# urbste/MultiCol-SLAM

Hardware: NVIDIA B200
Metric: Mfeatures/s extract+match (higher is better)
Workload: dtype u8

## Files before the change

multicol_slam_b200/csrc/describe_kernel.cu:

```cuda
#include <cstdlib>
#include <cstring>
#include <vector>

#include "cam_model.cuh"
#include "kernels.h"
#include "mcs_common.cuh"

namespace mcs {

__constant__ signed char c_pairs[2048];
__device__ float2 g_patf[1024];
__constant__ signed char c_disc_u[848], c_disc_v[848];

__device__ __forceinline__ float fast_atan2_deg(float y, float x) {
    const float s = (float)(180.0 / 3.14159265358979323846);
    const float p1 = 0.9997878412794807f * s, p3 = -0.3258083974640975f * s;
    const float p5 = 0.1555786518463281f * s, p7 = -0.04432655554792128f * s;
    const float ax = fabsf(x), ay = fabsf(y);
    float a, c, c2;
    if (ax >= ay) {
        c = __fdiv_rn(ay, __fadd_rn(ax, (float)2.2204460492503131e-16));
        c2 = __fmul_rn(c, c);
        a = __fmul_rn(__fadd_rn(__fmul_rn(__fadd_rn(__fmul_rn(__fadd_rn(__fmul_rn(p7, c2), p5), c2), p3), c2), p1), c);
    } else {
// ... 233 lines not shown
                tu = (u - uk) - mu; tv = (v - vk) - mv;
                ru = (tu + kMagic) - kMagic; rv = (tv + kMagic) - kMagic;
                bad |= !(fabs(tu - ru) < 0.5 - kT1RepairGuard) || !(fabs(tv - rv) < 0.5 - kT1RepairGuard);
            }
            bad |= !(fabs(tu) < (double)kPatchR + 0.4) || !(fabs(tv) < (double)kPatchR + 0.4);
            int ix = (int)ru, iy = (int)rv;
            ix = min(max(ix, -kPatchR), kPatchR); iy = min(max(iy, -kPatchR), kPatchR);
            smp[e2] = patch[pofs + iy * kPatchS + ix];
        }
        out |= (unsigned)(smp[0] < smp[1]) << (j >> 1);
    }
    if (lane_valid && (bad || worst_tau >= __double2hiint(1.0))) *fail = 1;
    return out;
}

struct __align__(16) WarpCtx {
    float t1[16];
    double ukx, uky, a_base, ca[3], sa[3];
    const double* row;
    int kx, ky, oidx, b, level;
    uint32_t c;
    float angle;
};
template <int PPL , int MINB = MCS_K3_MINB>
__global__ void __launch_bounds__(kDescWarps * 32, MINB)
describe_kernel(const PyramidGeom* __restrict__ geom, const DescribeArgs args, const mcs_ocam* __restrict__ cams,
                const DistortLut* __restrict__ luts, const int* __restrict__ cam_of_image,
                const uint32_t* __restrict__ sel_xys, const int* __restrict__ sel_count,
                mcs_keypoint* __restrict__ kps_out, uint8_t* __restrict__ desc_out, uint8_t* __restrict__ dmask_out,
                int* __restrict__ counts_out, const int capacity, const int n_images) {
    __shared__ mcs_ocam s_cam[kDescWarps];
    __shared__ WarpCtx s_ctx[kDescWarps];
    __shared__ __align__(8) float2 s_patf[PPL * 32];
    extern __shared__ __align__(8) float2 s_park_dyn[];
    __shared__ __align__(16) uint8_t s_patch[kDescWarps][(2 * kPatchR + 1) * kPatchS];
    const int ds = geom->desc_size;
#pragma unroll
    for (int i = threadIdx.x; i < PPL * 32; i += kDescWarps * 32) s_patf[i] = g_patf[i];
    __syncthreads();

    const int lane = threadIdx.x & 31, wib = threadIdx.x >> 5;
    const int warp_global = (blockIdx.x * blockDim.x + threadIdx.x) >> 5;
    const int sel_total = geom->sel_total;
    const int b = warp_global / sel_total;
    if (b >= n_images) return;
    const int slot = warp_global - b * sel_total;
    const int L = geom->nlevels;
    int level = 0, off = 0;
    for (int l = 0; l < L; ++l)
        if (slot >= geom->lv[l].sel_off) level = l;
    for (int l = 0; l < level; ++l) off += sel_count[b * L + l];
    const LevelGeom& g = geom->lv[level];
    const int p = slot - g.sel_off;
    const int cnt = sel_count[b * L + level];
    if (slot == 0 && lane == 0) {
        int tot = 0;
        for (int l = 0; l < L; ++l) tot += sel_count[b * L + l];
        counts_out[b] = min(tot, capacity);
    }
    if (p >= cnt) return;
    const int oidx = off + p;
    if (oidx >= capacity) return;
    const uint32_t c = sel_xys[(size_t)b * sel_total + slot];
    const int kx = corner_x(c), ky = corner_y(c);
    const uint8_t* uimg = args.lvl[level] + (size_t)b * g.img_bytes;
    const uint8_t* bimg = args.blur[level] + (size_t)b * g.img_bytes;
    const int pitch = g.pitch;

    uint8_t* patch = s_patch[wib];
    const int x0 = (kx - kPatchR) & ~3;
    {
        const int half = lane >> 4, w = lane & 15;
        const uint32_t* gp = (const uint32_t*)(bimg + (size_t)(ky - kPatchR + half) * pitch + x0) + w;
        uint32_t* sp = (uint32_t*)(patch + half * kPatchS) + w;
#pragma unroll
        for (int k0 = 0; k0 < 26; k0 += 13) {
            uint32_t t[13];
#pragma unroll
            for (int k = 0; k < 13; ++k) {
                const int r = half + 2 * (k0 + k);
                t[k] = (w < 15 && r < 2 * kPatchR + 1) ? __ldg(gp + (size_t)(k0 + k) * (pitch / 2)) : 0u;
            }
#pragma unroll
            for (int k = 0; k < 13; ++k) {
                const int r = half + 2 * (k0 + k);
                if (w < 15 && r < 2 * kPatchR + 1) sp[(k0 + k) * (2 * kPatchS / 4)] = t[k];
            }
        }
    }
    const int pofs = kPatchR * kPatchS + (kx - x0);

    int m10 = 0, m01 = 0;
#if MCS_K3_V3
    {
        constexpr int kIcS = 40;
        uint8_t* ic = reinterpret_cast<uint8_t*>(s_park_dyn + wib * (PPL * 32));
        const int xs = (kx - kHalfPatch) & ~3;
        {
            const int rr = lane / 10, w = lane - rr * 10;
            const uint32_t* gp = (const uint32_t*)(uimg + (size_t)(ky - kHalfPatch + rr) * pitch + xs) + w;
            uint32_t* sp = (uint32_t*)(ic + rr * kIcS) + w;
            uint32_t t[11];
#pragma unroll
            for (int k = 0; k < 11; ++k) t[k] = (lane < 30) ? __ldg(gp + (size_t)k * 3 * (pitch / 4)) : 0u;
#pragma unroll
            for (int k = 0; k < 11; ++k) if (lane < 30) sp[k * 3 * (kIcS / 4)] = t[k];
        }
        __syncwarp();
        const int u = lane - kHalfPatch;
        const int au = u < 0 ? -u : u;
        const int vm = c_disc_u[au];
        const uint8_t* col = ic + kHalfPatch * kIcS + (kx - kHalfPatch - xs) + lane;
        int sum = col[0];
#pragma unroll
        for (int k = 1; k <= kHalfPatch; ++k) {
            const int a = col[k * kIcS], bb = col[-k * kIcS];
            if (vm >= k) { sum += a + bb; m01 += k * (a - bb); }
        }
        m10 = u * sum;
        const int um = c_disc_u[kHalfPatch];
        if (lane < 2 * um + 1) {
            const int v = lane - um;
            const int val = ic[(kHalfPatch + v) * kIcS + (kx - kHalfPatch - xs) + 2 * kHalfPatch];
            m10 += kHalfPatch * val;
            m01 += v * val;
        }
#pragma unroll
        for (int o = 16; o; o >>= 1) {
            m10 += __shfl_xor_sync(0xffffffffu, m10, o);
            m01 += __shfl_xor_sync(0xffffffffu, m01, o);
        }
        __syncwarp();
    }
#else
    {
        const uint8_t* ctr = uimg + (size_t)ky * pitch + kx;
        const int u = lane - kHalfPatch;
        const int au = u < 0 ? -u : u;
        const int vm = c_disc_u[au];
#pragma unroll 11
        for (int v = -kHalfPatch; v <= kHalfPatch; ++v) {
            const int val = (v >= -vm && v <= vm) ? (int)ctr[v * pitch + u] : 0;
            m10 += u * val;
            m01 += v * val;
        }
        if (lane < 2 * c_disc_u[kHalfPatch] + 1) {
            const int v = lane - c_disc_u[kHalfPatch];
            const int val = ctr[v * pitch + kHalfPatch];
            m10 += kHalfPatch * val;
            m01 += v * val;
        }
#pragma unroll
        for (int o = 16; o; o >>= 1) {
            m10 += __shfl_xor_sync(0xffffffffu, m10, o);
            m01 += __shfl_xor_sync(0xffffffffu, m01, o);
        }
    }
#endif
    const float angle = fast_atan2_deg((float)m01, (float)m10);

    WarpCtx& cx = s_ctx[wib];
    const int ci = cam_of_image[b];
    const bool masks = geom->learn_masks != 0, dbrief = geom->do_dbrief != 0 || masks;
    const int npat = masks ? 3 : 1;
    {
        double a0, s0, c0;
        if (masks) a0 = (double)__fdiv_rn(angle, 57.2957763671875f);
        else a0 = (double)__fmul_rn(angle, 0.01745329238474369f);
        sincos(a0, &s0, &c0);
        if (lane == 0) {
            cx.kx = kx; cx.ky = ky; cx.oidx = oidx; cx.b = b; cx.level = level; cx.c = c; cx.angle = angle; cx.a_base = a0;
            const double c20 = 0.93969262078590838405, s20 = 0.34202014332566873304;
            cx.ca[0] = c0; cx.sa[0] = s0;
            cx.ca[1] = fma(c0, c20, -s0 * s20); cx.sa[1] = fma(s0, c20, c0 * s20);
            cx.ca[2] = fma(c0, c20, s0 * s20);  cx.sa[2] = fma(s0, c20, -c0 * s20);
        }
    }
    constexpr int BPL = PPL / 16;
    unsigned v0[BPL], vdiff[BPL];
#pragma unroll
    for (int bb = 0; bb < BPL; ++bb) { v0[bb] = 0u; vdiff[bb] = 0u; }
    auto put = [&](int qi, unsigned e ) {
#pragma unroll
        for (int bb = 0; bb < BPL; ++bb) {
            const unsigned v = (e >> (8 * bb)) & 0xFFu;
            if (qi == 0) v0[bb] = v; else vdiff[bb] |= v ^ v0[bb];
        }
    };
    __syncwarp();
    if (!dbrief) {
        const double ca0 = cx.ca[0], sa0 = cx.sa[0];
        int ix[PPL], iy[PPL];
        bool far = false;
#pragma unroll
        for (int j = 0; j < PPL; ++j) {
            const float2 pp = s_patf[j * 32 + lane];
            const double px = (double)pp.x, py = (double)pp.y;
            ix[j] = __double2int_rn(px * ca0 - py * sa0);
            iy[j] = __double2int_rn(px * sa0 + py * ca0);
            far |= (unsigned)(ix[j] + kPatchR) > 2u * kPatchR || (unsigned)(iy[j] + kPatchR) > 2u * kPatchR;
        }
        if (__any_sync(0xffffffffu, far)) {
            put(0, orb_pattern_global<PPL>(s_patf, ca0, sa0, lane, bimg, uimg, &g, kx, ky));
        } else {
            unsigned e = 0;
#pragma unroll
            for (int bb = 0; bb < BPL; ++bb) {
#pragma unroll
                for (int bit = 0; bit < 8; ++bit) {
                    const int j0 = 16 * bb + 2 * bit;
                    const int s0 = patch[pofs + iy[j0] * kPatchS + ix[j0]], s1 = patch[pofs + iy[j0 + 1] * kPatchS + ix[j0 + 1]];
                    e |= (unsigned)(s0 < s1) << (8 * bb + bit);
                }
            }
            put(0, e);
        }
    } else {
        if (lane < (int)(sizeof(mcs_ocam) / 8)) ((double*)&s_cam[wib])[lane] = ((const double*)&cams[ci])[lane];
        __syncwarp();
        const mcs_ocam& cam = s_cam[wib];
        const bool lane_valid = (PPL == 32) || (lane < ds);
        bool have_lut, t1, mform;
        {
            float q[kT1MCoef], K0f = 0.f, gkf = 0.f, s0f = 0.f, rk2f = 0.f, rkf = 0.f, auk = 0.f, avk = 0.f;
#pragma unroll
            for (int k = 0; k < kT1MCoef; ++k) q[k] = 0.f;
            const DistortLut lut = luts[ci];
            const float scale = g.scale;
            double ukx, uky;
            cam_undistort(cam, (double)__fmul_rn((float)kx, scale), (double)__fmul_rn((float)ky, scale), cam.pol[0], ukx, uky);
            const double rk = sqrt(ukx * ukx + uky * uky);
            have_lut = rk < (double)(lut.n - 1);
            const int ci_lut = have_lut ? __double2int_rn(rk) : 0;
            const double* row = lut.coef + (size_t)ci_lut * kLutStride;
            if (lane == 0) { cx.ukx = ukx; cx.uky = uky; cx.row = row; }
            t1 = MCS_K3_T1 && have_lut && rk >= kT1MinRadius && __ldg(row + 17) == 1.0;
            mform = MCS_K3_MFORM && t1 && __ldg(row + 23) == 1.0;
            if (mform) {
                const float2 c01 = __ldg((const float2*)(row + 19)), c23 = __ldg((const float2*)(row + 20));
                const float2 c45 = __ldg((const float2*)(row + 21)), c67 = __ldg((const float2*)(row + 22));
                q[0] = c01.x; q[1] = c01.y; q[2] = c23.x; q[3] = c23.y; q[4] = c45.x; q[5] = c45.y; q[6] = c67.x; q[7] = c67.y;
                const double inv_hw = 1.0 / t1m_halfwidth(ci_lut);
                const double tk = (rk * rk - t1m_centre(ci_lut)) * inv_hw;
                double pk = (double)q[7];
#pragma unroll
                for (int k = 6; k >= 0; --k) pk = fma(pk, tk, (double)q[k]);
                const double K0 = tk * pk;
                gkf = (float)(__ldg(row + 18) + K0);
                K0f = (float)K0; s0f = (float)tk; rk2f = (float)inv_hw;
                auk = (float)(cam.c * ukx + cam.d * uky); avk = (float)(cam.e * ukx + uky);
            } else if (t1) {
                const double Ri = __ldg(row + 12), q0d = __ldg(row + 13);
                const float2 c12 = __ldg((const float2*)(row + 14)), c34 = __ldg((const float2*)(row + 15)), c5x = __ldg((const float2*)(row + 16));
                q[1] = c12.x; q[2] = c12.y; q[3] = c34.x; q[4] = c34.y; q[5] = c5x.x; q[6] = 0.f; q[7] = 0.f;
                const double s0 = (rk - (double)ci_lut) * (1.0 / (double)kT1Scale);
                double pk = (double)q[5];
                pk = fma(pk, s0, (double)q[4]); pk = fma(pk, s0, (double)q[3]); pk = fma(pk, s0, (double)q[2]);
                pk = fma(pk, s0, (double)q[1]); pk = fma(pk, s0, q0d);
                const double dRk = s0 * pk;
                const double gk = (Ri + dRk) / rk;
                q[0] = (float)(q0d - gk * (double)kT1Scale);
                K0f = (float)(dRk - gk * (rk - (double)ci_lut));
                gkf = (float)gk; s0f = (float)s0;
                rk2f = (float)(rk * rk); rkf = (float)rk;
                auk = (float)(cam.c * ukx + cam.d * uky); avk = (float)(cam.e * ukx + uky);
            }
            if (lane == 0) {
                float4* tp = reinterpret_cast<float4*>(cx.t1);
                tp[0] = make_float4(q[0], q[1], q[2], q[3]); tp[1] = make_float4(q[4], q[5], q[6], q[7]);
                tp[2] = make_float4(K0f, gkf, s0f, rk2f);    tp[3] = make_float4(rkf, auk, avk, 0.f);
            }
        }
        __syncwarp();
#pragma unroll 1
        for (int qi = 0; qi < npat; ++qi) {
            bool done = false;
            float2* park = s_park_dyn + wib * (PPL * 32);
            if (t1) {
                float nx, ny, axx, axy, ayx, ayy;
                {
                    const double caq = cx.ca[qi], saq = cx.sa[qi], ukx = cx.ukx, uky = cx.uky;
                    nx = (float)(2.0 * (ukx * caq + uky * saq)); ny = (float)(2.0 * (uky * caq - ukx * saq));
                    axx = (float)(cam.c * caq + cam.d * saq); axy = (float)(cam.d * caq - cam.c * saq);
                    ayx = (float)(cam.e * caq + saq); ayy = (float)(caq - cam.e * saq);
                }
                float su = 0.f, sv = 0.f;
                {
                const float4* tp = reinterpret_cast<const float4*>(cx.t1);
                const float4 tA = tp[0], tB = tp[1], tC = tp[2], tD = tp[3];
                const float q[kT1MCoef] = {tA.x, tA.y, tA.z, tA.w, tB.x, tB.y, tB.z, tB.w};
                const float K0f = tC.x, gkf = tC.y, s0f = tC.z, rk2f = tC.w, rkf = tD.x, auk = tD.y, avk = tD.z;
                if (mform) {
#pragma unroll kT1Unroll1
                    for (int j = 0; j < PPL; ++j) {
                        const float2 pp = s_patf[j * 32 + lane];
                        const float n = fmaf(pp.x, nx, fmaf(pp.y, ny, fmaf(pp.x, pp.x, pp.y * pp.y)));
                        const float t = fmaf(n, rk2f, s0f);
                        float pl = q[kT1MCoef - 1];
#pragma unroll
                        for (int k = kT1MCoef - 2; k >= 0; --k) pl = fmaf(pl, t, q[k]);
                        const float dg = fmaf(t, pl, -K0f);
                        const float g = gkf + dg;
                        const float du = fmaf(g, fmaf(pp.x, axx, pp.y * axy), dg * auk);
                        const float dv = fmaf(g, fmaf(pp.x, ayx, pp.y * ayy), dg * avk);
                        park[j * 32 + lane] = make_float2(du, dv);
                        if (lane_valid) { su += du; sv += dv; }
                    }
                } else
#pragma unroll 4
                for (int j = 0; j < PPL; ++j) {
                    const float2 pp = s_patf[j * 32 + lane];
                    const float n = fmaf(pp.x, nx, fmaf(pp.y, ny, fmaf(pp.x, pp.x, pp.y * pp.y)));
                    const float r2 = rk2f + n;
                    float y, z;
                    asm("rsqrt.approx.ftz.f32 %0, %1;" : "=f"(y) : "f"(r2));
                    y = fmaf(0.5f * y, fmaf(-r2 * y, y, 1.f), y);
                    const float w = fmaf(r2, y, rkf);
                    asm("rcp.approx.ftz.f32 %0, %1;" : "=f"(z) : "f"(w));
                    z = fmaf(z, fmaf(-w, z, 1.f), z);
                    const float delta = n * z;
                    const float sp = fmaf(delta, 1.f / kT1Scale, s0f);
                    float pl = q[5];
                    pl = fmaf(pl, sp, q[4]); pl = fmaf(pl, sp, q[3]); pl = fmaf(pl, sp, q[2]);
                    pl = fmaf(pl, sp, q[1]); pl = fmaf(pl, sp, q[0]);
                    const float dg = fmaf(sp, pl, -K0f) * y;
                    const float g = gkf + dg;
                    const float du = fmaf(g, fmaf(pp.x, axx, pp.y * axy), dg * auk);
                    const float dv = fmaf(g, fmaf(pp.x, ayx, pp.y * ayy), dg * avk);
                    park[j * 32 + lane] = make_float2(du, dv);
                    if (lane_valid) { su += du; sv += dv; }
                }
                }
                const double inv_n = 1.0 / (double)(16 * ds);
                bool flag = false;
#if MCS_K3_V3
                flag = !(fabsf(su) < 500.f) | !(fabsf(sv) < 500.f);
                const int iu = __reduce_add_sync(0xffffffffu, flag ? 0 : __float2int_rn(su * 131072.f));
                const int iv = __reduce_add_sync(0xffffffffu, flag ? 0 : __float2int_rn(sv * 131072.f));
                const float mu = (float)((double)iu * (inv_n * (1.0 / 131072.0))), mv = (float)((double)iv * (inv_n * (1.0 / 131072.0)));
                float wf = 0.f, wt = 0.f;
#else
                double sud = (double)su, svd = (double)sv;
#pragma unroll
                for (int o = 16; o; o >>= 1) {
                    sud += __shfl_xor_sync(0xffffffffu, sud, o);
                    svd += __shfl_xor_sync(0xffffffffu, svd, o);
                }
                const float mu = (float)(sud * inv_n), mv = (float)(svd * inv_n);
#endif
                constexpr float kMagicF = 12582912.f;
                unsigned bits = 0;
#pragma unroll kT1Unroll2
                for (int j = 0; j < PPL; j += 2) {
                    int smp[2];
#pragma unroll
                    for (int e2 = 0; e2 < 2; ++e2) {
                        const float2 c = park[(j + e2) * 32 + lane];
                        const float tu = c.x - mu, tv = c.y - mv;
                        const float mu_r = tu + kMagicF, mv_r = tv + kMagicF;
                        const float fu = tu - (mu_r - kMagicF), fv = tv - (mv_r - kMagicF);
#if MCS_K3_V3
                        wf = fmaxf(wf, fmaxf(fabsf(fu), fabsf(fv)));
                        wt = fmaxf(wt, fmaxf(fabsf(tu), fabsf(tv)));
#else
                        flag |= !(fabsf(fu) < 0.5f - kT1Guard) | !(fabsf(fv) < 0.5f - kT1Guard) | !(fabsf(tu) < (float)kPatchR + 0.4f) |
                                !(fabsf(tv) < (float)kPatchR + 0.4f);
#endif
                        const int ix = __float_as_int(mu_r) - 0x4B400000, iy = __float_as_int(mv_r) - 0x4B400000;
                        const int ofs = min(max(iy * kPatchS + ix, -(kPatchR * kPatchS + kPatchR)), kPatchR * kPatchS + kPatchR);
                        smp[e2] = patch[pofs + ofs];
                    }
                    bits |= (unsigned)(smp[0] < smp[1]) << (j >> 1);
// ... 31 lines not shown
                if (args.tier_stats && lane == 0) atomicAdd(args.tier_stats + (exact ? 3 : 2), 1ull);
                put(qi, e);
            }
        }
    }
    {
        const int bo = cx.b, oo = cx.oidx;
#pragma unroll
        for (int bb = 0; bb < BPL; ++bb) {
            const int byte = lane + 32 * bb;
            if (byte < ds) {
                desc_out[((size_t)bo * capacity + oo) * ds + byte] = (uint8_t)v0[bb];
                if (dmask_out) dmask_out[((size_t)bo * capacity + oo) * ds + byte] = (uint8_t)(masks ? (~vdiff[bb] & 0xFFu) : 0u);
            }
        }
        if (lane == 0) {
            const int lv = cx.level, kxo = cx.kx, kyo = cx.ky;
            const LevelGeom& go = geom->lv[lv];
            const float scale = go.scale;
            mcs_keypoint k;
            k.x = lv ? __fmul_rn((float)kxo, scale) : (float)kxo;
            k.y = lv ? __fmul_rn((float)kyo, scale) : (float)kyo;
            k.size = go.patch_size; k.angle = cx.angle; k.response = (float)corner_s(cx.c);
            k.octave = lv; k.class_id = -1;
            kps_out[(size_t)bo * capacity + oo] = k;
        }
    }
}

cudaError_t upload_constants(const signed char* pairs, const signed char* du, const signed char* dv) {
    cudaError_t e = cudaMemcpyToSymbol(c_pairs, pairs, 2048);
    if (e != cudaSuccess) return e;
    {
        std::vector<float2> pf(1024);
        for (int i = 0; i < 1024; ++i) {
            const int j = i >> 5, ln = i & 31, byte = ln + 32 * (j >> 4), pt = 16 * byte + (j & 15);
            pf[i] = make_float2((float)pairs[2 * pt], (float)pairs[2 * pt + 1]);
        }
        e = cudaMemcpyToSymbol(g_patf, pf.data(), sizeof(float2) * 1024);
        if (e != cudaSuccess) return e;
    }
// ... 133 lines not shown
                long double pv = (long double)af[NM - 1];
                for (int t = NM - 2; t >= 0; --t) pv = pv * tv + (long double)af[t];
                werr = std::max(werr, fabsl(tv * pv - (G_exact(cm + hm * tv) - Gc)));
            }
            if (werr * ((long double)i + 1.0L) < 1e-6L) {
                e[18] = (double)Gc;
                std::memcpy(&e[19], af, sizeof(float) * NM);
                e[23] = 1.0;
            }
        }
    }
}

cudaError_t launch_describe(const PyramidGeom& G, const PyramidGeom* G_dev, int n_images, const DescribeArgs& args,
                            const mcs_ocam* cams, const DistortLut* luts, const int* cam_of_image, const uint32_t* sel_xys,
                            const int* sel_count, mcs_keypoint* kps, uint8_t* desc, uint8_t* dmask, int* counts, int capacity,
                            cudaStream_t st) {
    const long long warps = (long long)n_images * G.sel_total;
    const int blocks = (int)std::max<long long>(1, (warps + kDescWarps - 1) / kDescWarps);
    const size_t park16 = (size_t)kDescWarps * 16 * 32 * sizeof(float2), park32 = 2 * park16;
    if (G.desc_size > 32) {
        cudaError_t e = cudaFuncSetAttribute(describe_kernel<32>, cudaFuncAttributeMaxDynamicSharedMemorySize, (int)park32);
        if (e != cudaSuccess) return e;
    }
    if (G.desc_size <= 32)
        describe_kernel<16><<<blocks, kDescWarps * 32, park16, st>>>(G_dev, args, cams, luts, cam_of_image, sel_xys, sel_count, kps, desc,
                                                               dmask, counts, capacity, n_images);
    else
        describe_kernel<32><<<blocks, kDescWarps * 32, park32, st>>>(G_dev, args, cams, luts, cam_of_image, sel_xys, sel_count, kps, desc,
                                                               dmask, counts, capacity, n_images);
    return cudaGetLastError();
}

}
```

multicol_slam_b200/csrc/kernels.h:

```cpp
#pragma once
#include <vector>

#include "mcs_common.cuh"

namespace mcs {

struct DescribeArgs {
    const uint8_t* lvl[kMaxLevels];
    const uint8_t* blur[kMaxLevels];
    unsigned long long* tier_stats = nullptr;
};

cudaError_t upload_constants(const signed char* pairs, const signed char* du, const signed char* dv);
void launch_pyr_fast(const PyramidGeom& G, int level, int n_images, const uint8_t* src, size_t src_img_bytes,
                     uint8_t* dst, uint8_t* dst_blur, const uint8_t* mask0, int mask_w, size_t mask_bytes,
                     const int* cam_of_image, const uint8_t* tile_flags, uint32_t* raw, int* raw_count, cudaStream_t st);
cudaError_t launch_octree(const PyramidGeom& G, const PyramidGeom* G_dev, int n_images, const uint32_t* raw,
                          const int* raw_count, uint16_t* node_of, uint32_t* sel_xys, int* sel_count, int* status,
                          cudaStream_t st, int level_lo = 0, int level_count = -1);
struct DistortLut {
    const double* coef;
    int n;
    double inv_h;
};
void build_distort_lut(const mcs_ocam& cam, std::vector<double>& coef, int& n_out);
cudaError_t launch_describe(const PyramidGeom& G, const PyramidGeom* G_dev, int n_images, const DescribeArgs& args,
                            const mcs_ocam* cams, const DistortLut* luts, const int* cam_of_image, const uint32_t* sel_xys,
                            const int* sel_count, mcs_keypoint* kps, uint8_t* desc, uint8_t* dmask, int* counts, int capacity,
                            cudaStream_t st);

cudaError_t launch_hamming_topk(const uint8_t* q, const uint8_t* qmask, int nq, const uint8_t* d, const uint8_t* dmask,
                                int nd, const uint8_t* db_skip, int dim, int K, unsigned bound, int* topk_idx, int* topk_dist,
                                cudaStream_t st);
cudaError_t launch_hamming_stream(const uint8_t* desc, const uint8_t* dmask, const int* counts, int img_lo, int img_count,
                                  int n_cams, int capacity, int dim, int K, unsigned bound, int* out_idx, int* out_dist, cudaStream_t st);
inline cudaError_t keep_pool_memory() {
    static bool done[64] = {};
    int dev = 0;
    cudaError_t e = cudaGetDevice(&dev);
    if (e != cudaSuccess || dev < 0 || dev >= 64 || done[dev]) return e;
    cudaMemPool_t pool;
    e = cudaDeviceGetDefaultMemPool(&pool, dev);
    if (e != cudaSuccess) return e;
    unsigned long long keep = ~0ull;
// ... 56 lines not shown
```

multicol_slam_b200/csrc/mcs_api.cu:

```cuda
#include <algorithm>
#include <climits>
#include <cmath>
#include <cstdio>
#include <cstring>
#include <mutex>
#include <string>
#include <vector>

#include "cam_model.cuh"
#include "kernels.h"
#include "mcs_common.cuh"

using namespace mcs;

namespace {

thread_local std::string g_err;
int fail(int code, const std::string& msg) { g_err = msg; return code; }

#define CK(expr)                                                                                       \
    do {                                                                                               \
        cudaError_t e__ = (expr);                                                                      \
        if (e__ != cudaSuccess) {                                                                      \
            cudaGetLastError();                                                                        \
// ... 43 lines not shown
    int geom_w = 0, geom_h = 0, geom_stride = 0;
    DevBuf<uint8_t> lut_blob;
    DevBuf<PyramidGeom> G_dev;

    int B_cap = 0;
    DevBuf<uint8_t> in_images;
    DevBuf<uint8_t> lvl[kMaxLevels], blur[kMaxLevels];
    DevBuf<uint8_t> masks;
    DevBuf<mcs_ocam> cams;
    DevBuf<int> cam_of_image, coi_all;
    const int* coi_last = nullptr;
    DevBuf<uint32_t> raw;
    DevBuf<uint16_t> node_of;
    DevBuf<int> raw_count, sel_count, status, counts;
    DevBuf<uint32_t> sel_xys;
    DevBuf<mcs_keypoint> kps;
    DevBuf<uint8_t> desc, dmask;
    int last_n_images = 0;
    DevBuf<int> match_idx, match_dist, m12, nmat, redo;
    DevBuf<uint8_t> in_tight;
    cudaStream_t s_copy = nullptr, s_out = nullptr, s_match = nullptr;
    std::vector<mcs_ocam> lut_cams;
    std::vector<uint8_t> masks_host;
    std::vector<int16_t> h_mx[kMaxLevels], h_my[kMaxLevels];
    DevBuf<uint8_t> tile_flags;
    bool tile_flags_valid = false;
    DevBuf<double> lut_coef;
    DevBuf<DistortLut> luts;
    uint8_t* pin_in = nullptr;  size_t pin_in_bytes = 0;
    uint8_t* pin_out = nullptr; size_t pin_out_bytes = 0;
// ... 138 lines not shown
}

int ensure_batch(mcs_extractor* ex, int B) {
    if (B <= ex->B_cap) return MCS_OK;
    const PyramidGeom& G = ex->G;
    for (int l = 0; l < G.nlevels; ++l) {
        CK(ex->lvl[l].ensure(G.lv[l].img_bytes * B + 256));
        CK(ex->blur[l].ensure(G.lv[l].img_bytes * B + 256));
    }
    CK(ex->cam_of_image.ensure(B));
    CK(ex->raw.ensure(G.raw_total * B));
    CK(ex->node_of.ensure(G.raw_total * B));
    CK(ex->raw_count.ensure((size_t)B * G.nlevels));
    CK(ex->sel_count.ensure((size_t)B * G.nlevels));
    CK(ex->sel_xys.ensure((size_t)B * G.sel_total));
    CK(ex->status.ensure(1));
    ex->B_cap = B;
    return MCS_OK;
}

int upload_small_inputs(mcs_extractor* ex, int W, int H, const uint8_t* masks, const mcs_ocam* cams, int n_cams, cudaStream_t st) {
    CK(ex->masks.ensure((size_t)n_cams * W * H));
    CK(ex->cams.ensure(n_cams));
    const size_t mbytes = (size_t)n_cams * W * H;
    if (ex->masks_host.size() != mbytes || std::memcmp(ex->masks_host.data(), masks, mbytes) != 0) {
        CK(cudaStreamSynchronize(st));
        ex->masks_host.assign(masks, masks + mbytes);
        CK(cudaMemcpyAsync(ex->masks.p, ex->masks_host.data(), mbytes, cudaMemcpyHostToDevice, st));
        ex->tile_flags_valid = false;
    }
// ... 64 lines not shown
        const uint8_t* src = l ? ex->lvl[l - 1].p : images_dev;
        const size_t src_bytes = l ? G.lv[l - 1].img_bytes : (size_t)stride * H;
        launch_pyr_fast(G, l, n_images, src, src_bytes, ex->lvl[l].p, ex->blur[l].p, ex->masks.p, W, (size_t)W * H,
                        coi_d, ex->tile_flags.p, ex->raw.p, ex->raw_count.p, st);
    }
    CK(cudaGetLastError());
    if (ex->profiling) CK(cudaEventRecord(ex->ev[1], st));
    CK(launch_octree(G, ex->G_dev.p, n_images, ex->raw.p, ex->raw_count.p, ex->node_of.p, ex->sel_xys.p, ex->sel_count.p,
                     ex->status.p, st));
    CK(cudaGetLastError());
    if (ex->profiling) CK(cudaEventRecord(ex->ev[2], st));
    DescribeArgs a;
    for (int l = 0; l < kMaxLevels; ++l) { a.lvl[l] = ex->lvl[l].p; a.blur[l] = ex->blur[l].p; }
    a.tier_stats = ex->tier_on ? ex->tier.p : nullptr;
    CK(launch_describe(G, ex->G_dev.p, n_images, a, ex->cams.p, ex->luts.p, coi_d, ex->sel_xys.p, ex->sel_count.p,
                       kps_dev, desc_dev, dmask_dev, counts_dev, capacity, st));
    if (ex->profiling) CK(cudaEventRecord(ex->ev[3], st));
    ex->last_n_images = n_images;
    return MCS_OK;
}

int prepare_inputs(mcs_extractor* ex, int n_images, int W, int H, int stride, const uint8_t* masks, const mcs_ocam* cams, int n_cams,
                   const int* cam_of_image, cudaStream_t st, bool first_chunk, const int* coi_dev, const int** coi_d) {
    if (n_cams < 1 || n_cams > 64) return fail(MCS_ERR_INVALID, "n_cams must be in [1,64]");
    for (int i = 0; i < n_images; ++i)
        if (cam_of_image[i] < 0 || cam_of_image[i] >= n_cams) return fail(MCS_ERR_INVALID, "cam_of_image out of range");
    int rc = build_geometry(ex, W, H, stride);
    if (rc) return rc;
    rc = ensure_batch(ex, n_images);
    if (rc) return rc;
    if (first_chunk) {
// ... 146 lines not shown
    if (cudaStreamCreateWithFlags(&ex->stream, cudaStreamNonBlocking) != cudaSuccess) {
        delete ex;
        return fail(MCS_ERR_CUDA, "cudaStreamCreate failed");
    }
    *out = ex;
    return MCS_OK;
}

void mcs_extractor_destroy(mcs_extractor* ex) {
    if (!ex) return;
    cudaSetDevice(ex->device);
    ex->lut_blob.release(); ex->G_dev.release(); ex->in_images.release();
    for (int l = 0; l < kMaxLevels; ++l) { ex->lvl[l].release(); ex->blur[l].release(); }
    ex->masks.release(); ex->cams.release(); ex->cam_of_image.release(); ex->coi_all.release(); ex->raw.release(); ex->node_of.release();
    ex->raw_count.release(); ex->sel_count.release(); ex->status.release(); ex->counts.release(); ex->sel_xys.release();
    ex->kps.release(); ex->desc.release(); ex->dmask.release();
    if (ex->sf_exec) cudaGraphExecDestroy(ex->sf_exec);
    if (ex->pin_in) cudaFreeHost(ex->pin_in);
    if (ex->pin_out) cudaFreeHost(ex->pin_out);
    ex->match_idx.release(); ex->match_dist.release(); ex->m12.release(); ex->nmat.release(); ex->redo.release(); ex->lut_coef.release(); ex->luts.release(); ex->tier.release(); ex->tile_flags.release();
    for (int i = 0; i < 4; ++i) if (ex->ev[i]) cudaEventDestroy(ex->ev[i]);
    ex->in_tight.release();
    if (ex->s_copy) cudaStreamDestroy(ex->s_copy);
    if (ex->s_match) cudaStreamDestroy(ex->s_match);
    if (ex->s_out) cudaStreamDestroy(ex->s_out);
    if (ex->stream) cudaStreamDestroy(ex->stream);
    delete ex;
}

int mcs_extractor_get_info(const mcs_extractor* ex, mcs_extractor_info* info) {
// ... 550 lines not shown
```

Measured before the change: 56.35.

## Split describe into setup kernel computing orientation/camera context and compact describe pass

Result: faster. 59.25 (median of 6 runs) (+5.1%).

```diff
diff --git a/multicol_slam_b200/csrc/describe_kernel.cu b/multicol_slam_b200/csrc/describe_kernel.cu
--- a/multicol_slam_b200/csrc/describe_kernel.cu
+++ b/multicol_slam_b200/csrc/describe_kernel.cu
@@ -271,23 +271,211 @@
     return out;
 }
 
-struct __align__(16) WarpCtx {
+struct __align__(16) DescribeCtx {
     float t1[16];
+    float pat[3][6];
     double ukx, uky, a_base, ca[3], sa[3];
     const double* row;
-    int kx, ky, oidx, b, level;
-    uint32_t c;
-    float angle;
+    int kx, ky, oidx, b, level, ci;
+    int flags;
+    int pad[3];
 };
+static_assert(sizeof(DescribeCtx) == kDescribeCtxBytes && sizeof(DescribeCtx) % 8 == 0 && sizeof(DescribeCtx) <= 256,
+              "the context is copied by one 8-byte load per lane");
+constexpr int kCtxHaveLut = 1, kCtxT1 = 2, kCtxMform = 4;
+
+constexpr int kSetupWarps = 4;
+constexpr int kIcS = 40;
+
+__global__ void __launch_bounds__(kSetupWarps * 32)
+describe_setup_kernel(const PyramidGeom* __restrict__ geom, const DescribeArgs args, const mcs_ocam* __restrict__ cams,
+                      const DistortLut* __restrict__ luts, const int* __restrict__ cam_of_image,
+                      const uint32_t* __restrict__ sel_xys, const int* __restrict__ sel_count, DescribeCtx* __restrict__ ctx,
+                      mcs_keypoint* __restrict__ kps_out, int* __restrict__ counts_out, const int stride, const int capacity,
+                      const int n_images) {
+    __shared__ __align__(4) uint8_t s_ic[kSetupWarps][(2 * kHalfPatch + 1) * kIcS];
+    __shared__ mcs_ocam s_cam[kSetupWarps];
+    const int lane = threadIdx.x & 31, wib = threadIdx.x >> 5;
+    const int chunks = (stride + 31) >> 5;
+    const int warp_global = (blockIdx.x * blockDim.x + threadIdx.x) >> 5;
+    const int b = warp_global / chunks;
+    if (b >= n_images) return;
+    const int oidx = (warp_global - b * chunks) * 32 + lane;
+    const int L = geom->nlevels;
+    int tot = 0, level = 0, off = 0;
+    for (int l = 0; l < L; ++l) {
+        if (oidx >= tot) { level = l; off = tot; }
+        tot += sel_count[b * L + l];
+    }
+    const int n = min(tot, capacity);
+    if (oidx == 0) counts_out[b] = n;
+    const bool valid = oidx < n;
+    const LevelGeom& g = geom->lv[level];
+    const int sel_total = geom->sel_total;
+    const uint32_t c = valid ? sel_xys[(size_t)b * sel_total + g.sel_off + (oidx - off)] : 0u;
+    const int kx = corner_x(c), ky = corner_y(c);
+
+    const int nk = __popc(__ballot_sync(0xffffffffu, valid));
+    int my_m10 = 0, my_m01 = 0;
+    uint8_t* ic = s_ic[wib];
+    const int rr = lane / 10, wl = lane - rr * 10;
+    uint32_t t[11];
+    auto load_disc = [&](int k) {
+        const int kxk = __shfl_sync(0xffffffffu, kx, k), kyk = __shfl_sync(0xffffffffu, ky, k), lk = __shfl_sync(0xffffffffu, level, k);
+        const LevelGeom& gk = geom->lv[lk];
+        const int pitch = gk.pitch;
+        const uint8_t* uimg = args.lvl[lk] + (size_t)b * gk.img_bytes;
+        const int xs = (kxk - kHalfPatch) & ~3;
+        const uint32_t* gp = (const uint32_t*)(uimg + (size_t)(kyk - kHalfPatch + rr) * pitch + xs) + wl;
+#pragma unroll
+        for (int i = 0; i < 11; ++i) t[i] = (lane < 30) ? __ldg(gp + (size_t)i * 3 * (pitch / 4)) : 0u;
+    };
+    if (nk > 0) load_disc(0);
+    for (int k = 0; k < nk; ++k) {
+        {
+            uint32_t* sp = (uint32_t*)(ic + rr * kIcS) + wl;
+#pragma unroll
+            for (int i = 0; i < 11; ++i) if (lane < 30) sp[i * 3 * (kIcS / 4)] = t[i];
+        }
+        __syncwarp();
+        if (k + 1 < nk) load_disc(k + 1);
+        const int kxk = __shfl_sync(0xffffffffu, kx, k);
+        const int cofs = kxk - kHalfPatch - ((kxk - kHalfPatch) & ~3);
+        int m10 = 0, m01 = 0;
+        const int u = lane - kHalfPatch;
+        const int au = u < 0 ? -u : u;
+        const int vm = c_disc_u[au];
+        const uint8_t* col = ic + kHalfPatch * kIcS + cofs + lane;
+        int sum = col[0];
+#pragma unroll
+        for (int kk = 1; kk <= kHalfPatch; ++kk) {
+            const int a = col[kk * kIcS], bb = col[-kk * kIcS];
+            if (vm >= kk) { sum += a + bb; m01 += kk * (a - bb); }
+        }
+        m10 = u * sum;
+        const int um = c_disc_u[kHalfPatch];
+        if (lane < 2 * um + 1) {
+            const int v = lane - um;
+            const int val = ic[(kHalfPatch + v) * kIcS + cofs + 2 * kHalfPatch];
+            m10 += kHalfPatch * val;
+            m01 += v * val;
+        }
+#pragma unroll
+        for (int o = 16; o; o >>= 1) {
+            m10 += __shfl_xor_sync(0xffffffffu, m10, o);
+            m01 += __shfl_xor_sync(0xffffffffu, m01, o);
+        }
+        if (lane == k) { my_m10 = m10; my_m01 = m01; }
+        __syncwarp();
+    }
+    const bool masks = geom->learn_masks != 0, dbrief = geom->do_dbrief != 0 || masks;
+    const int ci = valid ? cam_of_image[b] : 0;
+    if (dbrief && lane < (int)(sizeof(mcs_ocam) / 8)) ((double*)&s_cam[wib])[lane] = ((const double*)&cams[cam_of_image[b]])[lane];
+    __syncwarp();
+    if (!valid) return;
+    const float angle = fast_atan2_deg((float)my_m01, (float)my_m10);
+    {
+        mcs_keypoint k;
+        k.x = level ? __fmul_rn((float)kx, g.scale) : (float)kx;
+        k.y = level ? __fmul_rn((float)ky, g.scale) : (float)ky;
+        k.size = g.patch_size; k.angle = angle; k.response = (float)corner_s(c);
+        k.octave = level; k.class_id = -1;
+        kps_out[(size_t)b * capacity + oidx] = k;
+    }
+
+    DescribeCtx& cx = ctx[(size_t)b * stride + oidx];
+    cx.kx = kx; cx.ky = ky; cx.oidx = oidx; cx.b = b; cx.level = level; cx.ci = ci;
+    cx.pad[0] = cx.pad[1] = cx.pad[2] = 0;
+    double ca[3], sa[3];
+    {
+        double a0, s0, c0;
+        if (masks) a0 = (double)__fdiv_rn(angle, 57.2957763671875f);
+        else a0 = (double)__fmul_rn(angle, 0.01745329238474369f);
+        sincos(a0, &s0, &c0);
+        cx.a_base = a0;
+        const double c20 = 0.93969262078590838405, s20 = 0.34202014332566873304;
+        ca[0] = c0; sa[0] = s0;
+        ca[1] = fma(c0, c20, -s0 * s20); sa[1] = fma(s0, c20, c0 * s20);
+        ca[2] = fma(c0, c20, s0 * s20);  sa[2] = fma(s0, c20, -c0 * s20);
+#pragma unroll
+        for (int qi = 0; qi < 3; ++qi) { cx.ca[qi] = ca[qi]; cx.sa[qi] = sa[qi]; }
+    }
+    if (!dbrief) {
+        cx.flags = 0;
+        cx.ukx = cx.uky = 0.0; cx.row = nullptr;
+        float4* zp = reinterpret_cast<float4*>(cx.t1);
+#pragma unroll
+        for (int i = 0; i < 8; ++i) zp[i] = make_float4(0.f, 0.f, 0.f, 0.f);
+        reinterpret_cast<float2*>(cx.t1)[16] = make_float2(0.f, 0.f);
+        return;
+    }
+    const mcs_ocam& cam = s_cam[wib];
+    float q[kT1MCoef], K0f = 0.f, gkf = 0.f, s0f = 0.f, rk2f = 0.f, rkf = 0.f, auk = 0.f, avk = 0.f;
+#pragma unroll
+    for (int k = 0; k < kT1MCoef; ++k) q[k] = 0.f;
+    const DistortLut lut = luts[ci];
+    const float scale = g.scale;
+    double ukx, uky;
+    cam_undistort(cam, (double)__fmul_rn((float)kx, scale), (double)__fmul_rn((float)ky, scale), cam.pol[0], ukx, uky);
+    const double rk = sqrt(ukx * ukx + uky * uky);
+    const bool have_lut = rk < (double)(lut.n - 1);
+    const int ci_lut = have_lut ? __double2int_rn(rk) : 0;
+    const double* row = lut.coef + (size_t)ci_lut * kLutStride;
+    cx.ukx = ukx; cx.uky = uky; cx.row = row;
+    const bool t1 = MCS_K3_T1 && have_lut && rk >= kT1MinRadius && __ldg(row + 17) == 1.0;
+    const bool mform = MCS_K3_MFORM && t1 && __ldg(row + 23) == 1.0;
+    cx.flags = (have_lut ? kCtxHaveLut : 0) | (t1 ? kCtxT1 : 0) | (mform ? kCtxMform : 0);
+    if (mform) {
+        const float2 c01 = __ldg((const float2*)(row + 19)), c23 = __ldg((const float2*)(row + 20));
+        const float2 c45 = __ldg((const float2*)(row + 21)), c67 = __ldg((const float2*)(row + 22));
+        q[0] = c01.x; q[1] = c01.y; q[2] = c23.x; q[3] = c23.y; q[4] = c45.x; q[5] = c45.y; q[6] = c67.x; q[7] = c67.y;
+        const double inv_hw = 1.0 / t1m_halfwidth(ci_lut);
+        const double tk = (rk * rk - t1m_centre(ci_lut)) * inv_hw;
+        double pk = (double)q[7];
+#pragma unroll
+        for (int k = 6; k >= 0; --k) pk = fma(pk, tk, (double)q[k]);
+        const double K0 = tk * pk;
+        gkf = (float)(__ldg(row + 18) + K0);
+        K0f = (float)K0; s0f = (float)tk; rk2f = (float)inv_hw;
+        auk = (float)(cam.c * ukx + cam.d * uky); avk = (float)(cam.e * ukx + uky);
+    } else if (t1) {
+        const double Ri = __ldg(row + 12), q0d = __ldg(row + 13);
+        const float2 c12 = __ldg((const float2*)(row + 14)), c34 = __ldg((const float2*)(row + 15)), c5x = __ldg((const float2*)(row + 16));
+        q[1] = c12.x; q[2] = c12.y; q[3] = c34.x; q[4] = c34.y; q[5] = c5x.x; q[6] = 0.f; q[7] = 0.f;
+        const double s0 = (rk - (double)ci_lut) * (1.0 / (double)kT1Scale);
+        double pk = (double)q[5];
+        pk = fma(pk, s0, (double)q[4]); pk = fma(pk, s0, (double)q[3]); pk = fma(pk, s0, (double)q[2]);
+        pk = fma(pk, s0, (double)q[1]); pk = fma(pk, s0, q0d);
+        const double dRk = s0 * pk;
+        const double gk = (Ri + dRk) / rk;
+        q[0] = (float)(q0d - gk * (double)kT1Scale);
+        K0f = (float)(dRk - gk * (rk - (double)ci_lut));
+        gkf = (float)gk; s0f = (float)s0;
+        rk2f = (float)(rk * rk); rkf = (float)rk;
+        auk = (float)(cam.c * ukx + cam.d * uky); avk = (float)(cam.e * ukx + uky);
+    }
+    {
+        float4* tp = reinterpret_cast<float4*>(cx.t1);
+        tp[0] = make_float4(q[0], q[1], q[2], q[3]); tp[1] = make_float4(q[4], q[5], q[6], q[7]);
+        tp[2] = make_float4(K0f, gkf, s0f, rk2f);    tp[3] = make_float4(rkf, auk, avk, 0.f);
+    }
+#pragma unroll
+    for (int qi = 0; qi < 3; ++qi) {
+        const double caq = ca[qi], saq = sa[qi];
+        float* pc = cx.pat[qi];
+        pc[0] = (float)(2.0 * (ukx * caq + uky * saq)); pc[1] = (float)(2.0 * (uky * caq - ukx * saq));
+        pc[2] = (float)(cam.c * caq + cam.d * saq);     pc[3] = (float)(cam.d * caq - cam.c * saq);
+        pc[4] = (float)(cam.e * caq + saq);             pc[5] = (float)(caq - cam.e * saq);
+    }
+}
+
 template <int PPL , int MINB = MCS_K3_MINB>
 __global__ void __launch_bounds__(kDescWarps * 32, MINB)
 describe_kernel(const PyramidGeom* __restrict__ geom, const DescribeArgs args, const mcs_ocam* __restrict__ cams,
-                const DistortLut* __restrict__ luts, const int* __restrict__ cam_of_image,
-                const uint32_t* __restrict__ sel_xys, const int* __restrict__ sel_count,
-                mcs_keypoint* __restrict__ kps_out, uint8_t* __restrict__ desc_out, uint8_t* __restrict__ dmask_out,
-                int* __restrict__ counts_out, const int capacity, const int n_images) {
+                const DescribeCtx* __restrict__ ctx, const int* __restrict__ counts, uint8_t* __restrict__ desc_out,
+                uint8_t* __restrict__ dmask_out, const int stride, const int capacity, const int n_images) {
     __shared__ mcs_ocam s_cam[kDescWarps];
-    __shared__ WarpCtx s_ctx[kDescWarps];
+    __shared__ DescribeCtx s_ctx[kDescWarps];
     __shared__ __align__(8) float2 s_patf[PPL * 32];
     extern __shared__ __align__(8) float2 s_park_dyn[];
     __shared__ __align__(16) uint8_t s_patch[kDescWarps][(2 * kPatchR + 1) * kPatchS];
@@ -298,29 +486,16 @@
 
     const int lane = threadIdx.x & 31, wib = threadIdx.x >> 5;
     const int warp_global = (blockIdx.x * blockDim.x + threadIdx.x) >> 5;
-    const int sel_total = geom->sel_total;
-    const int b = warp_global / sel_total;
+    const int b = warp_global / stride;
     if (b >= n_images) return;
-    const int slot = warp_global - b * sel_total;
-    const int L = geom->nlevels;
-    int level = 0, off = 0;
-    for (int l = 0; l < L; ++l)
-        if (slot >= geom->lv[l].sel_off) level = l;
-    for (int l = 0; l < level; ++l) off += sel_count[b * L + l];
+    const int oidx = warp_global - b * stride;
+    if (oidx >= counts[b]) return;
+    DescribeCtx& cx = s_ctx[wib];
+    if (lane < (int)(sizeof(DescribeCtx) / 8))
+        reinterpret_cast<uint2*>(&cx)[lane] = reinterpret_cast<const uint2*>(ctx + (size_t)b * stride + oidx)[lane];
+    __syncwarp();
+    const int level = cx.level, kx = cx.kx, ky = cx.ky;
     const LevelGeom& g = geom->lv[level];
-    const int p = slot - g.sel_off;
-    const int cnt = sel_count[b * L + level];
-    if (slot == 0 && lane == 0) {
-        int tot = 0;
-        for (int l = 0; l < L; ++l) tot += sel_count[b * L + l];
-        counts_out[b] = min(tot, capacity);
-    }
-    if (p >= cnt) return;
-    const int oidx = off + p;
-    if (oidx >= capacity) return;
-    const uint32_t c = sel_xys[(size_t)b * sel_total + slot];
-    const int kx = corner_x(c), ky = corner_y(c);
-    const uint8_t* uimg = args.lvl[level] + (size_t)b * g.img_bytes;
     const uint8_t* bimg = args.blur[level] + (size_t)b * g.img_bytes;
     const int pitch = g.pitch;
 
@@ -347,92 +522,8 @@
     }
     const int pofs = kPatchR * kPatchS + (kx - x0);
 
-    int m10 = 0, m01 = 0;
-#if MCS_K3_V3
-    {
-        constexpr int kIcS = 40;
-        uint8_t* ic = reinterpret_cast<uint8_t*>(s_park_dyn + wib * (PPL * 32));
-        const int xs = (kx - kHalfPatch) & ~3;
-        {
-            const int rr = lane / 10, w = lane - rr * 10;
-            const uint32_t* gp = (const uint32_t*)(uimg + (size_t)(ky - kHalfPatch + rr) * pitch + xs) + w;
-            uint32_t* sp = (uint32_t*)(ic + rr * kIcS) + w;
-            uint32_t t[11];
-#pragma unroll
-            for (int k = 0; k < 11; ++k) t[k] = (lane < 30) ? __ldg(gp + (size_t)k * 3 * (pitch / 4)) : 0u;
-#pragma unroll
-            for (int k = 0; k < 11; ++k) if (lane < 30) sp[k * 3 * (kIcS / 4)] = t[k];
-        }
-        __syncwarp();
-        const int u = lane - kHalfPatch;
-        const int au = u < 0 ? -u : u;
-        const int vm = c_disc_u[au];
-        const uint8_t* col = ic + kHalfPatch * kIcS + (kx - kHalfPatch - xs) + lane;
-        int sum = col[0];
-#pragma unroll
-        for (int k = 1; k <= kHalfPatch; ++k) {
-            const int a = col[k * kIcS], bb = col[-k * kIcS];
-            if (vm >= k) { sum += a + bb; m01 += k * (a - bb); }
-        }
-        m10 = u * sum;
-        const int um = c_disc_u[kHalfPatch];
-        if (lane < 2 * um + 1) {
-            const int v = lane - um;
-            const int val = ic[(kHalfPatch + v) * kIcS + (kx - kHalfPatch - xs) + 2 * kHalfPatch];
-            m10 += kHalfPatch * val;
-            m01 += v * val;
-        }
-#pragma unroll
-        for (int o = 16; o; o >>= 1) {
-            m10 += __shfl_xor_sync(0xffffffffu, m10, o);
-            m01 += __shfl_xor_sync(0xffffffffu, m01, o);
-        }
-        __syncwarp();
-    }
-#else
-    {
-        const uint8_t* ctr = uimg + (size_t)ky * pitch + kx;
-        const int u = lane - kHalfPatch;
-        const int au = u < 0 ? -u : u;
-        const int vm = c_disc_u[au];
-#pragma unroll 11
-        for (int v = -kHalfPatch; v <= kHalfPatch; ++v) {
-            const int val = (v >= -vm && v <= vm) ? (int)ctr[v * pitch + u] : 0;
-            m10 += u * val;
-            m01 += v * val;
-        }
-        if (lane < 2 * c_disc_u[kHalfPatch] + 1) {
-            const int v = lane - c_disc_u[kHalfPatch];
-            const int val = ctr[v * pitch + kHalfPatch];
-            m10 += kHalfPatch * val;
-            m01 += v * val;
-        }
-#pragma unroll
-        for (int o = 16; o; o >>= 1) {
-            m10 += __shfl_xor_sync(0xffffffffu, m10, o);
-            m01 += __shfl_xor_sync(0xffffffffu, m01, o);
-        }
-    }
-#endif
-    const float angle = fast_atan2_deg((float)m01, (float)m10);
-
-    WarpCtx& cx = s_ctx[wib];
-    const int ci = cam_of_image[b];
     const bool masks = geom->learn_masks != 0, dbrief = geom->do_dbrief != 0 || masks;
     const int npat = masks ? 3 : 1;
-    {
-        double a0, s0, c0;
-        if (masks) a0 = (double)__fdiv_rn(angle, 57.2957763671875f);
-        else a0 = (double)__fmul_rn(angle, 0.01745329238474369f);
-        sincos(a0, &s0, &c0);
-        if (lane == 0) {
-            cx.kx = kx; cx.ky = ky; cx.oidx = oidx; cx.b = b; cx.level = level; cx.c = c; cx.angle = angle; cx.a_base = a0;
-            const double c20 = 0.93969262078590838405, s20 = 0.34202014332566873304;
-            cx.ca[0] = c0; cx.sa[0] = s0;
-            cx.ca[1] = fma(c0, c20, -s0 * s20); cx.sa[1] = fma(s0, c20, c0 * s20);
-            cx.ca[2] = fma(c0, c20, s0 * s20);  cx.sa[2] = fma(s0, c20, -c0 * s20);
-        }
-    }
     constexpr int BPL = PPL / 16;
     unsigned v0[BPL], vdiff[BPL];
 #pragma unroll
@@ -458,7 +549,7 @@
             far |= (unsigned)(ix[j] + kPatchR) > 2u * kPatchR || (unsigned)(iy[j] + kPatchR) > 2u * kPatchR;
         }
         if (__any_sync(0xffffffffu, far)) {
-            put(0, orb_pattern_global<PPL>(s_patf, ca0, sa0, lane, bimg, uimg, &g, kx, ky));
+            put(0, orb_pattern_global<PPL>(s_patf, ca0, sa0, lane, bimg, args.lvl[level] + (size_t)b * g.img_bytes, &g, kx, ky));
         } else {
             unsigned e = 0;
 #pragma unroll
@@ -473,74 +564,23 @@
             put(0, e);
         }
     } else {
-        if (lane < (int)(sizeof(mcs_ocam) / 8)) ((double*)&s_cam[wib])[lane] = ((const double*)&cams[ci])[lane];
+        if (lane < (int)(sizeof(mcs_ocam) / 8)) ((double*)&s_cam[wib])[lane] = ((const double*)&cams[cx.ci])[lane];
         __syncwarp();
         const mcs_ocam& cam = s_cam[wib];
         const bool lane_valid = (PPL == 32) || (lane < ds);
-        bool have_lut, t1, mform;
-        {
-            float q[kT1MCoef], K0f = 0.f, gkf = 0.f, s0f = 0.f, rk2f = 0.f, rkf = 0.f, auk = 0.f, avk = 0.f;
-#pragma unroll
-            for (int k = 0; k < kT1MCoef; ++k) q[k] = 0.f;
-            const DistortLut lut = luts[ci];
-            const float scale = g.scale;
-            double ukx, uky;
-            cam_undistort(cam, (double)__fmul_rn((float)kx, scale), (double)__fmul_rn((float)ky, scale), cam.pol[0], ukx, uky);
-            const double rk = sqrt(ukx * ukx + uky * uky);
-            have_lut = rk < (double)(lut.n - 1);
-            const int ci_lut = have_lut ? __double2int_rn(rk) : 0;
-            const double* row = lut.coef + (size_t)ci_lut * kLutStride;
-            if (lane == 0) { cx.ukx = ukx; cx.uky = uky; cx.row = row; }
-            t1 = MCS_K3_T1 && have_lut && rk >= kT1MinRadius && __ldg(row + 17) == 1.0;
-            mform = MCS_K3_MFORM && t1 && __ldg(row + 23) == 1.0;
-            if (mform) {
-                const float2 c01 = __ldg((const float2*)(row + 19)), c23 = __ldg((const float2*)(row + 20));
-                const float2 c45 = __ldg((const float2*)(row + 21)), c67 = __ldg((const float2*)(row + 22));
-                q[0] = c01.x; q[1] = c01.y; q[2] = c23.x; q[3] = c23.y; q[4] = c45.x; q[5] = c45.y; q[6] = c67.x; q[7] = c67.y;
-                const double inv_hw = 1.0 / t1m_halfwidth(ci_lut);
-                const double tk = (rk * rk - t1m_centre(ci_lut)) * inv_hw;
-                double pk = (double)q[7];
-#pragma unroll
-                for (int k = 6; k >= 0; --k) pk = fma(pk, tk, (double)q[k]);
-                const double K0 = tk * pk;
-                gkf = (float)(__ldg(row + 18) + K0);
-                K0f = (float)K0; s0f = (float)tk; rk2f = (float)inv_hw;
-                auk = (float)(cam.c * ukx + cam.d * uky); avk = (float)(cam.e * ukx + uky);
-            } else if (t1) {
-                const double Ri = __ldg(row + 12), q0d = __ldg(row + 13);
-                const float2 c12 = __ldg((const float2*)(row + 14)), c34 = __ldg((const float2*)(row + 15)), c5x = __ldg((const float2*)(row + 16));
-                q[1] = c12.x; q[2] = c12.y; q[3] = c34.x; q[4] = c34.y; q[5] = c5x.x; q[6] = 0.f; q[7] = 0.f;
-                const double s0 = (rk - (double)ci_lut) * (1.0 / (double)kT1Scale);
-                double pk = (double)q[5];
-                pk = fma(pk, s0, (double)q[4]); pk = fma(pk, s0, (double)q[3]); pk = fma(pk, s0, (double)q[2]);
-                pk = fma(pk, s0, (double)q[1]); pk = fma(pk, s0, q0d);
-                const double dRk = s0 * pk;
-                const double gk = (Ri + dRk) / rk;
-                q[0] = (float)(q0d - gk * (double)kT1Scale);
-                K0f = (float)(dRk - gk * (rk - (double)ci_lut));
-                gkf = (float)gk; s0f = (float)s0;
-                rk2f = (float)(rk * rk); rkf = (float)rk;
-                auk = (float)(cam.c * ukx + cam.d * uky); avk = (float)(cam.e * ukx + uky);
-            }
-            if (lane == 0) {
-                float4* tp = reinterpret_cast<float4*>(cx.t1);
-                tp[0] = make_float4(q[0], q[1], q[2], q[3]); tp[1] = make_float4(q[4], q[5], q[6], q[7]);
-                tp[2] = make_float4(K0f, gkf, s0f, rk2f);    tp[3] = make_float4(rkf, auk, avk, 0.f);
-            }
-        }
-        __syncwarp();
+        const int flags = cx.flags;
+        const bool have_lut = flags & kCtxHaveLut, t1 = flags & kCtxT1, mform = flags & kCtxMform;
 #pragma unroll 1
         for (int qi = 0; qi < npat; ++qi) {
             bool done = false;
             float2* park = s_park_dyn + wib * (PPL * 32);
             if (t1) {
-                float nx, ny, axx, axy, ayx, ayy;
-                {
-                    const double caq = cx.ca[qi], saq = cx.sa[qi], ukx = cx.ukx, uky = cx.uky;
-                    nx = (float)(2.0 * (ukx * caq + uky * saq)); ny = (float)(2.0 * (uky * caq - ukx * saq));
-                    axx = (float)(cam.c * caq + cam.d * saq); axy = (float)(cam.d * caq - cam.c * saq);
-                    ayx = (float)(cam.e * caq + saq); ayy = (float)(caq - cam.e * saq);
-                }
+                const float* pc = cx.pat[qi];
+                unsigned ln;
+                asm volatile("mov.u32 %0, %%laneid;" : "=r"(ln));
+                const float2* pat_l = s_patf + ln;
+                float2* park_l = park + ln;
+                const float nx = pc[0], ny = pc[1], axx = pc[2], axy = pc[3], ayx = pc[4], ayy = pc[5];
                 float su = 0.f, sv = 0.f;
                 {
                 const float4* tp = reinterpret_cast<const float4*>(cx.t1);
@@ -550,7 +590,7 @@
                 if (mform) {
 #pragma unroll kT1Unroll1
                     for (int j = 0; j < PPL; ++j) {
-                        const float2 pp = s_patf[j * 32 + lane];
+                        const float2 pp = pat_l[j * 32];
                         const float n = fmaf(pp.x, nx, fmaf(pp.y, ny, fmaf(pp.x, pp.x, pp.y * pp.y)));
                         const float t = fmaf(n, rk2f, s0f);
                         float pl = q[kT1MCoef - 1];
@@ -560,13 +600,13 @@
                         const float g = gkf + dg;
                         const float du = fmaf(g, fmaf(pp.x, axx, pp.y * axy), dg * auk);
                         const float dv = fmaf(g, fmaf(pp.x, ayx, pp.y * ayy), dg * avk);
-                        park[j * 32 + lane] = make_float2(du, dv);
+                        park_l[j * 32] = make_float2(du, dv);
                         if (lane_valid) { su += du; sv += dv; }
                     }
                 } else
 #pragma unroll 4
                 for (int j = 0; j < PPL; ++j) {
-                    const float2 pp = s_patf[j * 32 + lane];
+                    const float2 pp = pat_l[j * 32];
                     const float n = fmaf(pp.x, nx, fmaf(pp.y, ny, fmaf(pp.x, pp.x, pp.y * pp.y)));
                     const float r2 = rk2f + n;
                     float y, z;
@@ -584,7 +624,7 @@
                     const float g = gkf + dg;
                     const float du = fmaf(g, fmaf(pp.x, axx, pp.y * axy), dg * auk);
                     const float dv = fmaf(g, fmaf(pp.x, ayx, pp.y * ayy), dg * avk);
-                    park[j * 32 + lane] = make_float2(du, dv);
+                    park_l[j * 32] = make_float2(du, dv);
                     if (lane_valid) { su += du; sv += dv; }
                 }
                 }
@@ -612,7 +652,7 @@
                     int smp[2];
 #pragma unroll
                     for (int e2 = 0; e2 < 2; ++e2) {
-                        const float2 c = park[(j + e2) * 32 + lane];
+                        const float2 c = park_l[(j + e2) * 32];
                         const float tu = c.x - mu, tv = c.y - mv;
                         const float mu_r = tu + kMagicF, mv_r = tv + kMagicF;
                         const float fu = tu - (mu_r - kMagicF), fv = tv - (mv_r - kMagicF);
@@ -674,17 +714,6 @@
                 if (dmask_out) dmask_out[((size_t)bo * capacity + oo) * ds + byte] = (uint8_t)(masks ? (~vdiff[bb] & 0xFFu) : 0u);
             }
         }
-        if (lane == 0) {
-            const int lv = cx.level, kxo = cx.kx, kyo = cx.ky;
-            const LevelGeom& go = geom->lv[lv];
-            const float scale = go.scale;
-            mcs_keypoint k;
-            k.x = lv ? __fmul_rn((float)kxo, scale) : (float)kxo;
-            k.y = lv ? __fmul_rn((float)kyo, scale) : (float)kyo;
-            k.size = go.patch_size; k.angle = cx.angle; k.response = (float)corner_s(cx.c);
-            k.octave = lv; k.class_id = -1;
-            kps_out[(size_t)bo * capacity + oo] = k;
-        }
     }
 }
 
@@ -848,9 +877,17 @@
 
 cudaError_t launch_describe(const PyramidGeom& G, const PyramidGeom* G_dev, int n_images, const DescribeArgs& args,
                             const mcs_ocam* cams, const DistortLut* luts, const int* cam_of_image, const uint32_t* sel_xys,
-                            const int* sel_count, mcs_keypoint* kps, uint8_t* desc, uint8_t* dmask, int* counts, int capacity,
-                            cudaStream_t st) {
-    const long long warps = (long long)n_images * G.sel_total;
+                            const int* sel_count, void* ctx, mcs_keypoint* kps, uint8_t* desc, uint8_t* dmask, int* counts,
+                            int capacity, cudaStream_t st) {
+    const int stride = std::min(capacity, G.sel_total);
+    DescribeCtx* cx = static_cast<DescribeCtx*>(ctx);
+    {
+        const long long warps = (long long)n_images * ((stride + 31) / 32);
+        const int blocks = (int)std::max<long long>(1, (warps + kSetupWarps - 1) / kSetupWarps);
+        describe_setup_kernel<<<blocks, kSetupWarps * 32, 0, st>>>(G_dev, args, cams, luts, cam_of_image, sel_xys, sel_count, cx, kps,
+                                                                   counts, stride, capacity, n_images);
+    }
+    const long long warps = (long long)n_images * stride;
     const int blocks = (int)std::max<long long>(1, (warps + kDescWarps - 1) / kDescWarps);
     const size_t park16 = (size_t)kDescWarps * 16 * 32 * sizeof(float2), park32 = 2 * park16;
     if (G.desc_size > 32) {
@@ -858,11 +895,9 @@
         if (e != cudaSuccess) return e;
     }
     if (G.desc_size <= 32)
-        describe_kernel<16><<<blocks, kDescWarps * 32, park16, st>>>(G_dev, args, cams, luts, cam_of_image, sel_xys, sel_count, kps, desc,
-                                                               dmask, counts, capacity, n_images);
+        describe_kernel<16><<<blocks, kDescWarps * 32, park16, st>>>(G_dev, args, cams, cx, counts, desc, dmask, stride, capacity, n_images);
     else
-        describe_kernel<32><<<blocks, kDescWarps * 32, park32, st>>>(G_dev, args, cams, luts, cam_of_image, sel_xys, sel_count, kps, desc,
-                                                               dmask, counts, capacity, n_images);
+        describe_kernel<32><<<blocks, kDescWarps * 32, park32, st>>>(G_dev, args, cams, cx, counts, desc, dmask, stride, capacity, n_images);
     return cudaGetLastError();
 }
 
diff --git a/multicol_slam_b200/csrc/kernels.h b/multicol_slam_b200/csrc/kernels.h
--- a/multicol_slam_b200/csrc/kernels.h
+++ b/multicol_slam_b200/csrc/kernels.h
@@ -24,10 +24,11 @@
     double inv_h;
 };
 void build_distort_lut(const mcs_ocam& cam, std::vector<double>& coef, int& n_out);
+constexpr size_t kDescribeCtxBytes = 256;
 cudaError_t launch_describe(const PyramidGeom& G, const PyramidGeom* G_dev, int n_images, const DescribeArgs& args,
                             const mcs_ocam* cams, const DistortLut* luts, const int* cam_of_image, const uint32_t* sel_xys,
-                            const int* sel_count, mcs_keypoint* kps, uint8_t* desc, uint8_t* dmask, int* counts, int capacity,
-                            cudaStream_t st);
+                            const int* sel_count, void* ctx, mcs_keypoint* kps, uint8_t* desc, uint8_t* dmask, int* counts,
+                            int capacity, cudaStream_t st);
 
 cudaError_t launch_hamming_topk(const uint8_t* q, const uint8_t* qmask, int nq, const uint8_t* d, const uint8_t* dmask,
                                 int nd, const uint8_t* db_skip, int dim, int K, unsigned bound, int* topk_idx, int* topk_dist,
diff --git a/multicol_slam_b200/csrc/mcs_api.cu b/multicol_slam_b200/csrc/mcs_api.cu
--- a/multicol_slam_b200/csrc/mcs_api.cu
+++ b/multicol_slam_b200/csrc/mcs_api.cu
@@ -81,6 +81,7 @@
     DevBuf<uint16_t> node_of;
     DevBuf<int> raw_count, sel_count, status, counts;
     DevBuf<uint32_t> sel_xys;
+    DevBuf<uint8_t> describe_ctx;
     DevBuf<mcs_keypoint> kps;
     DevBuf<uint8_t> desc, dmask;
     int last_n_images = 0;
@@ -249,6 +250,7 @@
     CK(ex->raw_count.ensure((size_t)B * G.nlevels));
     CK(ex->sel_count.ensure((size_t)B * G.nlevels));
     CK(ex->sel_xys.ensure((size_t)B * G.sel_total));
+    CK(ex->describe_ctx.ensure((size_t)B * G.sel_total * kDescribeCtxBytes));
     CK(ex->status.ensure(1));
     ex->B_cap = B;
     return MCS_OK;
@@ -343,7 +345,7 @@
     for (int l = 0; l < kMaxLevels; ++l) { a.lvl[l] = ex->lvl[l].p; a.blur[l] = ex->blur[l].p; }
     a.tier_stats = ex->tier_on ? ex->tier.p : nullptr;
     CK(launch_describe(G, ex->G_dev.p, n_images, a, ex->cams.p, ex->luts.p, coi_d, ex->sel_xys.p, ex->sel_count.p,
-                       kps_dev, desc_dev, dmask_dev, counts_dev, capacity, st));
+                       ex->describe_ctx.p, kps_dev, desc_dev, dmask_dev, counts_dev, capacity, st));
     if (ex->profiling) CK(cudaEventRecord(ex->ev[3], st));
     ex->last_n_images = n_images;
     return MCS_OK;
@@ -520,6 +522,7 @@
     for (int l = 0; l < kMaxLevels; ++l) { ex->lvl[l].release(); ex->blur[l].release(); }
     ex->masks.release(); ex->cams.release(); ex->cam_of_image.release(); ex->coi_all.release(); ex->raw.release(); ex->node_of.release();
     ex->raw_count.release(); ex->sel_count.release(); ex->status.release(); ex->counts.release(); ex->sel_xys.release();
+    ex->describe_ctx.release();
     ex->kps.release(); ex->desc.release(); ex->dmask.release();
     if (ex->sf_exec) cudaGraphExecDestroy(ex->sf_exec);
     if (ex->pin_in) cudaFreeHost(ex->pin_in);
```
